# ethnhe/FFB6D

Hardware: AMD Instinct MI355X
Metric: RGB-D frames/sec fwd (480x640, N=12288, bs=8) (higher is better)
Workload: dtype f32; 1 GPU; FFB6D forward incl. on-device 22-call KNN index pyramid; bs=8/GPU, N=12288 pts, 480x640 RGB-D, 22 classes, fp32, eval; global_batch=8, n_points=12288, index_dtype=int64, layout=pm, parallelism=dp1 (independent batches, one process per GPU, no process group)

## Files before the change

### ffb6d_amd/_lib.py

```python
import ctypes
import os

from . import build as _build

_c = ctypes
_vp, _i64, _i32, _sz = _c.c_void_p, _c.c_int64, _c.c_int, _c.c_size_t

SIGNATURES = {
    "ffb6d_last_error": (_c.c_char_p, []),
    "ffb6d_abi_version": (_c.c_int, []),
    "cpp_knn": (None, [_vp, _sz, _sz, _vp, _sz, _sz, _vp]),
    "cpp_knn_omp": (None, [_vp, _sz, _sz, _vp, _sz, _sz, _vp]),
    "cpp_knn_batch": (None, [_vp, _sz, _sz, _sz, _vp, _sz, _sz, _vp]),
    "cpp_knn_batch_omp": (None, [_vp, _sz, _sz, _sz, _vp, _sz, _sz, _vp]),
    "cpp_knn_batch_distance_pick": (None, [_vp, _sz, _sz, _sz, _vp, _sz, _sz, _vp]),
    "cpp_knn_batch_distance_pick_omp": (None, [_vp, _sz, _sz, _sz, _vp, _sz, _sz, _vp]),
    "ffb6d_knn_workspace_bytes": (_sz, [_i64, _i64, _i64, _i32]),
    "ffb6d_knn_batch_device": (_i32, [_vp, _vp, _i64, _i64, _i64, _i32, _vp, _vp, _vp, _vp, _sz, _vp]),
    "ffb6d_knn_prepared_bytes": (_sz, [_i64, _i64]),
    "ffb6d_knn_prepare_workspace_bytes": (_sz, [_i64, _i64]),
    "ffb6d_knn_prepare": (_i32, [_vp, _i64, _i64, _vp, _sz, _vp, _sz, _vp]),
    "ffb6d_knn_prepare_multi_workspace_bytes": (_sz, [_i32, _vp, _i64]),
    "ffb6d_knn_prepare_multi": (_i32, [_i32, _vp, _vp, _i64, _vp, _vp, _vp, _sz, _vp]),
    "ffb6d_knn_search_multi": (_i32, [_i32, _vp, _i64, _vp]),
    "ffb6d_knn_search_prepared": (_i32, [_vp, _vp, _vp, _i64, _i64, _i64, _i32, _vp, _vp, _vp, _vp]),
    "ffb6d_knn_set_pair_counter": (_i32, [_vp]),
    "ffb6d_knn_uses_pruning": (_i32, [_i64, _i64, _i64, _i32]),
    "ffb6d_random_sample_f32": (_i32, [_vp, _vp, _i32, _vp, _vp, _i64, _i64, _i64, _i64, _i32, _vp]),
    "ffb6d_random_sample_bwd_f32": (_i32, [_vp, _vp, _vp, _i64, _i64, _i64, _i64, _vp]),
    "ffb6d_nearest_interpolation_f32": (_i32, [_vp, _vp, _i32, _vp, _i64, _i64, _i64, _i64, _vp]),
    "ffb6d_nearest_interpolation_bwd_f32": (_i32, [_vp, _vp, _i32, _vp, _i64, _i64, _i64, _i64, _vp]),
    "ffb6d_gather_neighbour_f32": (_i32, [_vp, _vp, _i32, _vp, _i64, _i64, _i64, _i64, _i32, _vp]),
    "ffb6d_gather_neighbour_bwd_f32": (_i32, [_vp, _vp, _i32, _vp, _i64, _i64, _i64, _i64, _i32, _vp]),
    "ffb6d_relative_pos_encoding_f32": (_i32, [_vp, _vp, _i32, _vp, _i64, _i64, _i32, _vp]),
    "ffb6d_att_pool_f32": (_i32, [_vp, _vp, _vp, _i64, _i64, _i64, _i32, _vp]),
    "ffb6d_relative_pos_encoding_cm_f32": (_i32, [_vp, _vp, _i32, _vp, _i64, _i64, _i32, _vp]),
    "ffb6d_att_pool_bwd_f32": (_i32, [_vp, _vp, _vp, _vp, _vp, _i64, _i64, _i64, _i32, _vp]),
    "ffb6d_mlp_pm_f32": (_i32, [_vp, _vp, _vp, _i64, _i64, _vp, _i64, _vp, _i64, _i64, _vp, _i64, _vp, _i64, _i32, _i64, _vp,
                                _i64, _i64, _i64, _i32, _i32, _vp]),
    "ffb6d_mlp_pm_tile": (_i32, [_i64, _i64, _i64, _i32]),
    "ffb6d_mlp_pm_choice": (_i32, [_i64, _i64, _i64, _i64, _i32, _i32, _i32]),
    "ffb6d_mlp_pm_seq_plan": (_i32, [_i64, _i64]),
    "ffb6d_mlp_pm_batched_f32": (_i32, [_vp, _i64, _i64, _vp, _i64, _i64, _vp, _i64, _i64, _i64, _i32, _vp]),
    "ffb6d_wino_input_f32": (_i32, [_vp, _vp, _i64, _i64, _i64, _i64, _i64, _vp]),
    "ffb6d_wino_output_f32": (_i32, [_vp, _vp, _vp, _vp, _vp, _vp, _vp, _i64, _i64, _i64, _i64, _i64, _i32, _c.c_float, _vp]),
    "ffb6d_wino4_input_f32": (_i32, [_vp, _vp, _i64, _i64, _i64, _i64, _i64, _vp]),
    "ffb6d_wino4_output_f32": (_i32, [_vp, _vp, _vp, _vp, _vp, _vp, _vp, _i64, _i64, _i64, _i64, _i64, _i32, _c.c_float, _vp]),
    "ffb6d_wino4_conv_f32": (_i32, [_vp, _vp, _vp, _vp, _vp, _vp, _vp, _vp, _i64, _i64, _i64, _i64, _i64, _i32, _c.c_float, _i32, _vp]),
    "ffb6d_wino4_conv_form": (_i32, [_i64, _i64]),
    "ffb6d_mlp_pm_set_big_form": (None, [_i32]),
    "ffb6d_mlp_pm_set_seq_lin": (None, [_i32]),
    "ffb6d_att_pool_pm_f32": (_i32, [_vp, _vp, _i64, _i64, _vp, _i32, _vp, _i64, _i64, _vp, _i64, _i64, _i64, _i32, _vp]),
    "ffb6d_mlp_pm_bf16": (_i32, [_vp, _vp, _vp, _i64, _i64, _vp, _i64, _vp, _i64, _i64, _vp, _i64, _vp, _i64, _i32, _i64, _vp,
                                 _i64, _i64, _i64, _i32, _i32, _vp]),
    "ffb6d_att_pool_pm_bf16": (_i32, [_vp, _vp, _i64, _i64, _vp, _i32, _vp, _i64, _i64, _vp, _i64, _i64, _i64, _i32, _vp]),
    "ffb6d_random_sample_pm": (_i32, [_i32, _vp, _vp, _i32, _vp, _i64, _i64, _i64, _i64, _i32, _vp]),
    "ffb6d_gather_rows_pm": (_i32, [_i32, _vp, _vp, _i32, _vp, _i64, _i64, _i64, _i64, _vp]),
    "ffb6d_relative_pos_encoding_pm": (_i32, [_i32, _vp, _vp, _i32, _vp, _i64, _i64, _i32, _vp]),
    "ffb6d_affine_act_pm": (_i32, [_i32, _vp, _vp, _vp, _vp, _vp, _vp, _vp, _i64, _i64, _i32, _c.c_float, _vp]),
    "ffb6d_affine_relu_maxpool_pm": (_i32, [_i32, _vp, _vp, _vp, _vp, _i64, _i64, _i64, _i64, _vp]),
    "ffb6d_bilinear_resize_pm": (_i32, [_i32, _vp, _vp, _i64, _i64, _i64, _i64, _i64, _i64, _i32, _vp]),
    "ffb6d_mlp_chain3_pm_f32": (_i32, [_vp, _i64, _vp, _vp, _i32, _vp, _vp, _i32, _vp, _vp, _i32, _vp, _i64, _i64, _i64, _vp]),
    "ffb6d_mlp_chain3_pm_bf16": (_i32, [_vp, _i64, _vp, _vp, _i32, _vp, _vp, _i32, _vp, _vp, _i32, _vp, _i64, _i64, _i64, _vp]),
    "ffb6d_upsampled_patch_rows_pm": (_i32, [_i32, _vp, _vp, _i32, _vp, _i64, _i64, _i64, _i64, _i64, _i64, _i64, _vp]),
    "ffb6d_posenc_mlp_pm": (_i32, [_i32, _vp, _vp, _i32, _vp, _i64, _vp, _i32, _vp, _i64, _i64, _i32, _i64, _vp]),
    "ffb6d_lfa_pm": (_i32, [_i32, _i32, _vp, _i64, _vp, _i32, _vp, _i64, _vp, _i64, _vp, _i32, _vp, _vp, _i32, _vp, _vp, _vp, _i32, _vp, _i64,
# ... 163 lines not shown
```

### ffb6d_amd/forward_pm.py

```python
import torch
import torch.nn.functional as F

from . import _lib, ops, ops_pm, pyramid


def cached(mod, name, sources, build):
    key = tuple((t._version, t.data_ptr(), t.device) for t in sources)
    store = mod.__dict__.setdefault("_pm_cache", {})
    hit = store.get(name)
    if hit is None or hit[0] != key:
        with torch.no_grad():
            hit = (key, build())
        store[name] = hit
    return hit[1]


def _pad_k(w, k_to):
    if w.shape[1] == k_to:
        return w.contiguous()
    out = w.new_zeros(w.shape[0], k_to)
    out[:, :w.shape[1]] = w
    return out


# ... 55 lines not shown


def mlp(m, x1, x2=None, pad_k=None, **kw):
    w, b = folded(m, pad_k, x1.dtype)
    return ops_pm.mlp(x1, w, b, m.act_code, x2=x2, **kw)


def fc_weight(att, dt=F32):
    w = att.fc.weight
    return cached(att, "fc%s" % dt, [w], lambda: w.detach().reshape(w.shape[0], -1).to(dt).contiguous())


POSENC_FUSED = True
STEM_FUSED = True
LFA_FUSED = True
HEADS_SHARE_FIRST = True
HEADS_ALIGN_LAST = True
HEADS_ON_BOTH_STREAMS = True
HEADS_CHAIN_FUSED = True
GEMM_SEQ_FORM = True
GEMM_BIG_FORM = True
GEMM_SEQ_LIN = False
GEMM_SEQ_LIN_ONE = False
LFA_WIDTHS = (32, 64, 128, 256)


def folded_kc(m, dt, perm=False):
    def build():
        w, b = folded(m, dt=dt)
        return ops_pm.k_chunked(w, perm), b
    return cached(m, "kc%s%d" % (dt, perm), mlp_sources(m), build)


def building_block(bb, xyz, f_pc, nei):
    dt = f_pc.dtype
    if LFA_FUSED and 2 * f_pc.shape[-1] in LFA_WIDTHS and nei.shape[-1] == 16:
        w1, b1 = folded(bb.mlp1)
        a1, a2 = bb.att_pooling_1, bb.att_pooling_2
        wm1, bm1 = folded_kc(a1.mlp, dt)
        f_agg = ops_pm.lfa_half(1, xyz, nei, f_pc, w1, b1, bb.mlp1.act_code, fc_weight(a1, dt), wm1, bm1, a1.mlp.act_code)
        w2, b2 = folded(bb.mlp2, dt=dt)
        wm2, bm2 = folded_kc(a2.mlp, dt)
        return ops_pm.lfa_half(2, xyz, nei, f_agg, w1, b1, bb.mlp1.act_code, fc_weight(a2, dt), wm2, bm2, a2.mlp.act_code,
                               w2=w2, b2=b2, act2=bb.mlp2.act_code)
    if xyz.shape[-1] == 4:
        xyz = xyz[..., :3].contiguous()
# ... 20 lines not shown
    w, b = cached(rb, "res%d%s" % (kin, dt), mlp_sources(rb.mlp2) + mlp_sources(rb.shortcut), build)
    return ops_pm.mlp(f, w, b, ops.ACT_LEAKY, x2=feature)


def decode(stage, skip, p_emb, interp_idx):
    wa, wb, bias = split(stage, skip.shape[-1], skip.dtype)
    y = ops_pm.mlp(p_emb, wb)
    return ops_pm.mlp(skip, wa, bias, stage.act_code, gather=(y, interp_idx.reshape(interp_idx.shape[0], -1)))


def fusion_step(pre_p2r, fuse_p2r, pre_r2p, fuse_r2p, rgb0, p0, p2r_idx, r2p_idx, main=None, side=None, handover=None, tag=""):
    B, h, w_, c = rgb0.shape
    if main is None:
        main = side = torch.cuda.current_stream(rgb0.device)
    if handover is None:
        handover = lambda t, producer, consumer, tag=None: t
    handover(p0, side, main, "main waits for point stage " + tag)
    handover(rgb0, main, side, "side waits for colour stage " + tag)
    if side is not main:
        p2r_idx.record_stream(main)
    e = mlp(pre_p2r, p0)
    wa, wb, bias = split(fuse_p2r, c, rgb0.dtype)
    y = ops_pm.mlp(e, wb)
    rgb = ops_pm.mlp(rgb0, wa, bias, fuse_p2r.act_code, gather=(y, p2r_idx.reshape(B, -1)))
    with torch.cuda.stream(side):
        r2p = mlp(pre_r2p, ops_pm.random_sample(rgb0.view(B, h * w_, c), r2p_idx))
        p = mlp(fuse_r2p, p0, x2=r2p)
    return rgb, p


def conv(x, c):
    w = cached(c, "cl%s" % x.dtype, [c.weight],
               lambda: c.weight.detach().to(x.dtype).contiguous(memory_format=torch.channels_last))
    y = F.conv2d(x.permute(0, 3, 1, 2), w, None, c.stride, c.padding, c.dilation, c.groups)
    y = y.permute(0, 2, 3, 1)
    return y if y.is_contiguous() else y.contiguous()


TRUNK_WINOGRAD = True
TRUNK_WINOGRAD_MIN_CIN = 256


def wino_filter(w):
    G = torch.tensor([[1, 0, 0], [.5, .5, .5], [.5, -.5, .5], [0, 0, 1]], dtype=torch.float64, device=w.device)
    u = G @ w.detach().double() @ G.T
    return u.permute(2, 3, 0, 1).reshape(16, w.shape[0], w.shape[1]).float().contiguous()


def wino_weights(c):
    return cached(c, "wino", [c.weight], lambda: wino_filter(c.weight))


TRUNK_WINOGRAD_F4 = True


def wino4_filter(w):
    G = torch.tensor([[1 / 2, 0, 0], [-1 / 6, -1 / 6, -1 / 6], [1 / 6, -1 / 6, 1 / 6], [1 / 30, 1 / 15, 2 / 15],
                      [-16 / 15, 8 / 15, -4 / 15], [0, 0, 1 / 2]], dtype=torch.float64, device=w.device)
    u = G @ w.detach().double() @ G.T
    return u.permute(2, 3, 0, 1).reshape(36, w.shape[0], w.shape[1]).float().contiguous()


def wino4_weights(c):
    return cached(c, "wino4", [c.weight], lambda: wino4_filter(c.weight))


def wino_variant(B, H, W):
    if not TRUNK_WINOGRAD_F4:
        return 2
    return 4 if 36 * ops_pm.wino4_tiles(B, H, W)[1] < 16 * ops_pm.wino_tiles(B, H, W)[1] else 2


def wino_ok(c, x, m=None):
    if not TRUNK_WINOGRAD or x.dtype != torch.float32 or c.weight.dtype != torch.float32:
        return False
    if (c.kernel_size, c.stride, c.padding, c.dilation, c.groups) != ((3, 3), (1, 1), (1, 1), (1, 1), 1) or c.bias is not None \
            or c.padding_mode != "zeros":
        return False
    cout, cin = c.weight.shape[:2]
    if cin < TRUNK_WINOGRAD_MIN_CIN or cin < 128 or cin % 32 or cout % 4:
        return False
    B, H, W, _ = x.shape
    if m is None:
        m = wino_variant(B, H, W)
    planes, Tp = (m + 2) ** 2, (ops_pm.wino4_tiles if m == 4 else ops_pm.wino_tiles)(B, H, W)[1]
    lim = (1 << 31) - (1 << 20)
    return planes * (Tp + 256) * max(cin, cout) * 4 < lim and B * H * W * max(cin, cout) * 4 < lim and planes * cout * cin * 4 < lim


def conv_wino(x, c, scale, shift, residual=None, res_affine=None, m=None):
    if m is None:
        m = wino_variant(*x.shape[:3])
    x = x if x.is_contiguous() else x.contiguous()
    if m == 4:
        mm = ops_pm.mlp_batched(ops_pm.wino4_input(x), wino4_weights(c))
        return ops_pm.wino4_output(mm, x.shape[:3], scale, shift, act=ops.ACT_RELU, residual=residual, res_affine=res_affine)
    if m != 2:
        raise ValueError(f"conv_wino: m must be 2, 4 or None, got {m}")
    u = wino_weights(c)
    v = ops_pm.wino_input(x)
    mm = ops_pm.mlp_batched(v, u)
    return ops_pm.wino_output(mm, x.shape[:3], scale, shift, act=ops.ACT_RELU, residual=residual, res_affine=res_affine)


TRUNK_WINOGRAD_FUSED = True
TRUNK_WINOGRAD_FUSED_WIDTHS = frozenset({(64, 64), (128, 128), (128, 256)})


def wino_fused_ok(c, x):
    if not (TRUNK_WINOGRAD and TRUNK_WINOGRAD_FUSED) or x.dtype != torch.float32 or c.weight.dtype != torch.float32:
        return False
    if (c.kernel_size, c.stride, c.padding, c.dilation, c.groups) != ((3, 3), (1, 1), (1, 1), (1, 1), 1) or c.bias is not None \
            or c.padding_mode != "zeros":
        return False
    cout, cin = c.weight.shape[:2]
    if (cin, cout) not in TRUNK_WINOGRAD_FUSED_WIDTHS or cin not in ops_pm.WINO4_CONV_CIN or cout not in ops_pm.WINO4_CONV_COUT:
        return False
    B, H, W, _ = x.shape
# ... 31 lines not shown
        return conv_wino(y, rb.conv2, *ops.bn_fold(rb.bn2), residual=res, res_affine=res_affine)
    return ops_pm.affine_act_(y, *ops.bn_fold(rb.bn2), act=ops.ACT_RELU, residual=res, res_affine=res_affine)


def pyramid_pooling(pp, x):
    B, h, w_, C = x.shape
    sizes = [st[0].output_size[0] for st in pp.stages]
    bw = pp.bottleneck.weight

    def build():
        ch = pp.stages[0][1].weight.shape[0]
        wb = bw.detach().reshape(bw.shape[0], -1)
        prods = [(wb[:, i * ch:(i + 1) * ch] @ st[1].weight.detach().reshape(ch, ch)).contiguous()
                 for i, st in enumerate(pp.stages)]
        return prods, wb[:, len(pp.stages) * ch:].contiguous()
    prods, wx = cached(pp, "fold", [bw] + [st[1].weight for st in pp.stages], build)
    pooled = ops_pm.psp_pool(x, sizes)
    zs, off = [], 0
    for s, wl in zip(sizes, prods):
        zs.append(ops_pm.mlp(pooled[:, off:off + s * s].contiguous(), wl, role="cnn"))
        off += s * s
    prior = ops_pm.psp_prior_sum(torch.cat(zs, dim=1), sizes, (h, w_), dtype=x.dtype)
    wx = cached(pp, "wx%s" % x.dtype, [bw], lambda: wx.to(x.dtype))
    return ops_pm.mlp(x, wx, pp.bottleneck.bias.detach().float(), ops.ACT_RELU, add=prior, role="cnn")


UPCONV_FOLD = "auto"
UPCONV_FOLD_BF16 = True


def _fold_block(cin, dtype):
    if UPCONV_FOLD == "auto":
        return dtype == torch.float32 or UPCONV_FOLD_BF16
    return UPCONV_FOLD is None or cin in UPCONV_FOLD


def upconv_folded(ub, dt=F32):
    cv, bn, prelu = ub.conv[1], ub.conv[2], ub.conv[3]
    if prelu.weight.numel() != 1:
        raise NotImplementedError("per-channel PReLU in PSPUpsample")

    def build():
        scale = bn.weight.detach() * torch.rsqrt(bn.running_var + bn.eps)
        shift = bn.bias.detach() - bn.running_mean * scale
        if cv.bias is not None:
            shift = shift + scale * cv.bias.detach()
        w = cv.weight.detach() * scale[:, None, None, None]
        w9 = w.permute(2, 3, 0, 1).reshape(9 * w.shape[0], w.shape[1])
        return w9.to(dt).contiguous(), shift.float().contiguous(), float(prelu.weight.detach().item())
    src = [cv.weight, bn.weight, bn.bias, bn.running_mean, bn.running_var, prelu.weight] + ([cv.bias] if cv.bias is not None else [])
    return cached(ub, "fold9%s" % dt, src, build)


def up_block(ub, x):
    B, h, w_, cin = x.shape
    cv, bn, prelu = ub.conv[1], ub.conv[2], ub.conv[3]
    if _fold_block(cin, x.dtype) and cv.kernel_size == (3, 3) and cv.padding == (1, 1) \
            and cv.stride == (1, 1) and cv.dilation == (1, 1) and cv.groups == 1:
        w9, shift, slope = upconv_folded(ub, x.dtype)
        z = ops_pm.mlp(x, w9, role="cnn")
        return ops_pm.upconv_combine(z, shift, slope, (2 * h, 2 * w_))
    y = ops_pm.bilinear_resize(x, (2 * h, 2 * w_), align_corners=True)
    y = conv(y, cv)
    if prelu.weight.numel() != 1:
        raise NotImplementedError("per-channel PReLU in PSPUpsample")
    slope = cached(ub, "slope", [prelu.weight], lambda: float(prelu.weight.detach().item()))
    scale, shift = ops.bn_fold(bn)
    shift = cached(ub, "shift", [cv.bias, bn.weight, bn.bias, bn.running_mean, bn.running_var],
                   lambda: (shift + scale * cv.bias.detach()).contiguous())
    return ops_pm.affine_act_(y, scale, shift, act=ops.ACT_LEAKY, slope=slope)


def final_head(fh, x):
    cv = fh[0]
    w = cached(fh, "w%s" % x.dtype, [cv.weight], lambda: cv.weight.detach().reshape(cv.out_channels, -1).to(x.dtype).contiguous())
    return ops_pm.mlp(x, w, cv.bias.detach().float(), ops_pm.ACT_LOG_SOFTMAX, role="cnn")


LAST_STAGE_AT_CHOSEN = True


def last_stage_at_chosen(stage, x, choose):
    from . import model
# ... 284 lines not shown
```

### ffb6d_amd/ops_pm.py

```python
import torch

from . import _lib
from .ops import ACT_LEAKY, ACT_NONE, ACT_RELU, _idx, _need_gpu, _stream


def _dt(*ts):
    dts = {t.dtype for t in ts if t is not None}
    if len(dts) != 1 or next(iter(dts)) not in (torch.float32, torch.bfloat16):
        raise TypeError(f"row operands must all be float32 or all bfloat16, got {sorted(map(str, dts))}")
    return 1 if next(iter(dts)) == torch.bfloat16 else 0


def rows_view(x):
    C = x.shape[-1]
    x2 = x.reshape(-1, C)
    if x2.stride(1) != 1 or x2.data_ptr() % 16 or (x2.shape[0] > 1 and (x2.stride(0) * x2.element_size()) % 16):
        x2 = x2.contiguous()
    return x2, (x2.stride(0) if x2.shape[0] > 1 else C)


ACT_LOG_SOFTMAX = 3
MLP_SEQ_FORM = True
MLP_BIG_FORM = True
MLP_SEQ_LIN = 0
_big_form_set = _seq_lin_set = None


def _sync_big_form(lib):
    global _big_form_set, _seq_lin_set
    if _big_form_set is not MLP_BIG_FORM:
        lib.ffb6d_mlp_pm_set_big_form(int(MLP_BIG_FORM))
        _big_form_set = MLP_BIG_FORM
    if _seq_lin_set != MLP_SEQ_LIN:
        lib.ffb6d_mlp_pm_set_seq_lin(int(MLP_SEQ_LIN))
        _seq_lin_set = MLP_SEQ_LIN


def mlp(x1, w, bias=None, act=ACT_NONE, x2=None, add=None, gather=None, x1_gather=None, out=None, tile_hint=0, role="path"):
    _need_gpu(x1, w)
    lib = _lib.load()
    _sync_big_form(lib)
    dt = _dt(x1, w, x2, add, gather[0] if gather is not None else None, out)
    tdt = x1.dtype
    esz = x1.element_size()
    if bias is not None and bias.dtype != torch.float32:
        raise TypeError("bias stays float32 in both precisions")
    a, ld1 = rows_view(x1.detach())
    K1 = a.shape[1]
    xi, px, bits = None, 0, 0
    lead = x1.shape[:-1]
    if x1_gather is not None:
        if x1.dim() != 3 or x1_gather.dim() != 2 or x1_gather.shape[0] != x1.shape[0]:
            raise ValueError("x1_gather needs x1 [B,M,K1] and idx [B,P]")
        xi, bits = _idx(x1_gather.reshape(-1))
        px = x1.shape[1]
        lead = tuple(x1_gather.shape)
    rows = 1
    for n in lead:
        rows *= int(n)
    P = rows // lead[0] if (x1_gather is not None or gather is not None) and len(lead) else rows
    b, ld2, K2 = None, 0, 0
# ... 19 lines not shown
        if gi.numel() != rows or rows % B:
            raise ValueError("gather index must have one entry per output row")
        P = rows // B
    elif add is not None:
        y, ldy = rows_view(add.detach())
        if y.shape[0] != rows or y.shape[1] != Cout:
            raise ValueError(f"add {tuple(add.shape)} does not match the output [{rows}, {Cout}]")
    if out is None:
        out = torch.empty(tuple(lead) + (Cout,), dtype=tdt, device=x1.device)
    if out.stride(-1) != 1 or out.numel() != rows * Cout:
        raise ValueError("out must be [..., Cout] with contiguous channels")
    ldo = out.stride(-2) if out.dim() >= 2 and rows > 1 else Cout
    if out.dim() > 2 and any(out.stride(i) != out.stride(i + 1) * out.shape[i + 1] for i in range(out.dim() - 2)):
        raise ValueError("out must be row-regular (a channel slice of a contiguous row buffer is fine)")
    nbytes = esz * ((K1 + K2) * Cout + rows * (K1 + K2) + rows * Cout) + rows * (bits // 8) * ((gi is not None) + (xi is not None)) + \
        (esz * (y.shape[0] if gi is None else rows) * Cout if y is not None else 0)
    if tile_hint == 0 and not MLP_SEQ_FORM and not dt and \
            (lib.ffb6d_mlp_pm_choice(rows, Cout, K1, K2, int(act), 0, int(xi is not None)) & 255) == 8:
        tile_hint = 7
    if _lib.TRACER is not None:
        tile = (int(tile_hint) if tile_hint > 0 else lib.ffb6d_mlp_pm_choice(rows, Cout, K1, K2, int(act), int(dt), int(xi is not None))) & 255
    else:
        tile = 0
    with torch.cuda.device(x1.device), _lib.traced("mlp_pm", nbytes, (K1 + K2, Cout, rows, tile, dt, role)):
        rc = (lib.ffb6d_mlp_pm_bf16 if dt else lib.ffb6d_mlp_pm_f32)(w.data_ptr(), bias.data_ptr() if bias is not None else None,
                                  a.data_ptr(), K1, ld1, xi.data_ptr() if xi is not None else None, px,
                                  b.data_ptr() if b is not None else None, K2, ld2,
                                  y.data_ptr() if y is not None else None, ldy,
                                  gi.data_ptr() if gi is not None else None, py, bits, P,
                                  out.data_ptr(), ldo, rows, Cout, int(act), int(tile_hint), _stream(x1))
    _lib.check(rc, "ffb6d_mlp_pm_f32")
    return out


def mlp_batched(x, w, out=None, tile_hint=0):
    _need_gpu(x, w)
    lib = _lib.load()
    if x.dtype != torch.float32 or w.dtype != torch.float32 or (out is not None and out.dtype != torch.float32):
        raise TypeError("mlp_batched is float32 only")
    if x.dim() != 3 or w.dim() != 3 or w.shape[0] != x.shape[0] or w.shape[2] != x.shape[2] or not x.is_contiguous() or not w.is_contiguous():
        raise ValueError(f"mlp_batched needs contiguous x [G,R,K] and w [G,Cout,K], got {tuple(x.shape)} / {tuple(w.shape)}")
    G, R, K = x.shape
    Cout = w.shape[1]
    if out is None:
        out = torch.empty(G, R, Cout, dtype=torch.float32, device=x.device)
    if out.shape != (G, R, Cout) or not out.is_contiguous():
        raise ValueError("out must be contiguous [G, R, Cout]")
    if tile_hint == 0 and not MLP_SEQ_FORM:
        tile_hint = 7
    nbytes = 4 * G * (Cout * K + R * K + R * Cout)
    with torch.cuda.device(x.device), _lib.traced("mlp_pm_batched", nbytes, (K, Cout, G * R, (int(tile_hint) & 255) or 8, 0, "cnn")):
        rc = lib.ffb6d_mlp_pm_batched_f32(w.data_ptr(), Cout * K, R, x.data_ptr(), K, K, out.data_ptr(), Cout, G * R, Cout,
                                          int(tile_hint), _stream(x))
    _lib.check(rc, "ffb6d_mlp_pm_batched_f32")
    return out


def wino_tiles(B, H, W):
    T = B * ((H + 1) // 2) * ((W + 1) // 2)
    return T, -(-T // 128) * 128


def wino_input(x, out=None):
    _need_gpu(x)
    lib = _lib.load()
    if x.dtype != torch.float32 or x.dim() != 4 or not x.is_contiguous():
        raise ValueError("wino_input needs a contiguous float32 [B,H,W,C] map")
    B, H, W, C = x.shape
    T, Tp = wino_tiles(B, H, W)
    if out is None:
        out = torch.empty(16, Tp, C, dtype=torch.float32, device=x.device)
    if out.shape != (16, Tp, C) or not out.is_contiguous() or out.dtype != torch.float32:
        raise ValueError(f"out must be contiguous float32 [16, {Tp}, {C}]")
# ... 417 lines not shown
```

### include/ffb6d_ops.h

```cpp
#ifndef FFB6D_OPS_H_
#define FFB6D_OPS_H_

#include "ffb6d_knn.h"

#ifdef __cplusplus
extern "C" {
#endif

int ffb6d_random_sample_f32(const float* feat, const void* idx, int idx_bits,
                            float* out, int32_t* arg,
                            int64_t B, int64_t C, int64_t M, int64_t Np, int K,
                            ffb6d_stream_t stream);

int ffb6d_random_sample_bwd_f32(const float* grad_out, const int32_t* arg, float* grad_feat,
                                int64_t B, int64_t C, int64_t M, int64_t Np,
                                ffb6d_stream_t stream);

int ffb6d_nearest_interpolation_f32(const float* feat, const void* idx, int idx_bits,
                                    float* out,
                                    int64_t B, int64_t C, int64_t M, int64_t U,
                                    ffb6d_stream_t stream);

int ffb6d_nearest_interpolation_bwd_f32(const float* grad_out, const void* idx, int idx_bits,
                                        float* grad_feat,
// ... 30 lines not shown

int ffb6d_depth_normal(const void* depth_mm, int depth_is_u16, double fx, double fy, int kernel_size,
                       int distance_threshold, int difference_threshold, int point_into_surface, float* out, int64_t B,
                       int64_t H, int64_t W, ffb6d_stream_t stream);

size_t ffb6d_fill_missing_workspace_bytes(int64_t B, int64_t H, int64_t W);
int ffb6d_fill_missing_f32(const float* depth, double cam_scale, double scale_2_80m, float max_depth, float* out, int64_t B,
                           int64_t H, int64_t W, void* workspace, size_t workspace_bytes, ffb6d_stream_t stream);


int ffb6d_mlp_pm_f32(const float* w, const float* bias, const float* x1, int64_t k1, int64_t ld1, const void* x1_idx,
                     int64_t x1_rows_per_frame, const float* x2, int64_t k2, int64_t ld2, const float* y, int64_t ldy,
                     const void* y_idx, int64_t y_rows_per_frame, int idx_bits, int64_t rows_per_frame, float* out,
                     int64_t ldo, int64_t rows, int64_t cout, int act, int tile_hint, ffb6d_stream_t stream);

int ffb6d_mlp_pm_tile(int64_t rows, int64_t cout, int64_t K, int act);
int ffb6d_mlp_pm_choice(int64_t rows, int64_t cout, int64_t k1, int64_t k2, int act, int bf16, int x1_gathered);
int ffb6d_mlp_pm_seq_plan(int64_t rows, int64_t cout);
void ffb6d_mlp_pm_set_seq_lin(int on);
void ffb6d_mlp_pm_set_big_form(int on);

int ffb6d_mlp_pm_batched_f32(const float* w, int64_t w_stride, int64_t rows_per_w, const float* x, int64_t k, int64_t ld, float* out,
                             int64_t ldo, int64_t rows, int64_t cout, int tile_hint, ffb6d_stream_t stream);

int ffb6d_wino_input_f32(const float* x, float* v, int64_t B, int64_t H, int64_t W, int64_t C, int64_t Tp, ffb6d_stream_t stream);
int ffb6d_wino_output_f32(const float* m, const float* scale, const float* shift, const float* res, const float* rscale,
                          const float* rshift, float* out, int64_t B, int64_t H, int64_t W, int64_t O, int64_t Tp, int act, float slope,
                          ffb6d_stream_t stream);

int ffb6d_wino4_input_f32(const float* x, float* v, int64_t B, int64_t H, int64_t W, int64_t C, int64_t Tp, ffb6d_stream_t stream);
int ffb6d_wino4_output_f32(const float* m, const float* scale, const float* shift, const float* res, const float* rscale,
                           const float* rshift, float* out, int64_t B, int64_t H, int64_t W, int64_t O, int64_t Tp, int act, float slope,
                           ffb6d_stream_t stream);

int ffb6d_wino4_conv_f32(const float* x, const float* u, const float* scale, const float* shift, const float* res, const float* rscale,
                         const float* rshift, float* out, int64_t B, int64_t H, int64_t W, int64_t C, int64_t O, int act, float slope,
                         int form, ffb6d_stream_t stream);
int ffb6d_wino4_conv_form(int64_t C, int64_t O);

int ffb6d_att_pool_pm_f32(const float* w_fc, const float* f, int64_t c1, int64_t ldf, const void* nei, int idx_bits,
                          const float* g, int64_t c2, int64_t ldg, float* out, int64_t ldo, int64_t B, int64_t N, int K,
                          ffb6d_stream_t stream);

int ffb6d_mlp_pm_bf16(const void* w, const float* bias, const void* x1, int64_t k1, int64_t ld1, const void* x1_idx,
                      int64_t x1_rows_per_frame, const void* x2, int64_t k2, int64_t ld2, const void* y, int64_t ldy,
                      const void* y_idx, int64_t y_rows_per_frame, int idx_bits, int64_t rows_per_frame, void* out,
// ... 74 lines not shown
```

Measured before the change: 646.8 frames/s.

## Add split-bf16 (bf16x3) MFMA GEMM form for large fp32 pointwise and Winograd layers

Adds a new GEMM kernel that emulates fp32 matrix multiplies with three bf16 splits of each operand and six bf16 MFMA products, so fp32 layers can use the bf16 matrix cores. Weight splits are precomputed and cached per module. The activation split happens on the fly while staging into LDS, with double-buffered LDS DMA for the weights. It is routed to large-row layers (p2r fusion, PSP bottleneck, folded upconv, Winograd-4 batched GEMM) only where the existing chooser would pick tile 8. Dropping the lowest-order cross terms costs a little accuracy relative to true fp32, and the kernel uses a large LDS footprint.

```diff
diff --git a/ffb6d_amd/_lib.py b/ffb6d_amd/_lib.py
--- a/ffb6d_amd/_lib.py
+++ b/ffb6d_amd/_lib.py
@@ -42,6 +42,10 @@
     "ffb6d_mlp_pm_choice": (_i32, [_i64, _i64, _i64, _i64, _i32, _i32, _i32]),
     "ffb6d_mlp_pm_seq_plan": (_i32, [_i64, _i64]),
     "ffb6d_mlp_pm_batched_f32": (_i32, [_vp, _i64, _i64, _vp, _i64, _i64, _vp, _i64, _i64, _i64, _i32, _vp]),
+    "ffb6d_mlp_pm_split_w": (_i32, [_vp, _vp, _i64, _vp]),
+    "ffb6d_mlp_pm_split_f32": (_i32, [_vp, _vp, _vp, _i64, _i64, _vp, _i64, _vp, _i64, _i64, _vp, _i64, _vp, _i64, _i32, _i64, _vp,
+                                      _i64, _i64, _i64, _i32, _i32, _vp]),
+    "ffb6d_mlp_pm_split_batched_f32": (_i32, [_vp, _i64, _i64, _vp, _i64, _i64, _vp, _i64, _i64, _i64, _vp]),
     "ffb6d_wino_input_f32": (_i32, [_vp, _vp, _i64, _i64, _i64, _i64, _i64, _vp]),
     "ffb6d_wino_output_f32": (_i32, [_vp, _vp, _vp, _vp, _vp, _vp, _vp, _i64, _i64, _i64, _i64, _i64, _i32, _c.c_float, _vp]),
     "ffb6d_wino4_input_f32": (_i32, [_vp, _vp, _i64, _i64, _i64, _i64, _i64, _vp]),
diff --git a/ffb6d_amd/csrc/mlp_pm_split.hip b/ffb6d_amd/csrc/mlp_pm_split.hip
--- /dev/null
+++ b/ffb6d_amd/csrc/mlp_pm_split.hip
@@ -0,0 +1,297 @@
+#include <algorithm>
+
+#include "common.h"
+#include "ffb6d_ops.h"
+#include "mlp_pm_common.h"
+
+namespace ffb6d {
+namespace pm {
+namespace {
+
+constexpr int SP_BLK = 512;
+constexpr int SP_RB = 64;
+constexpr int SP_WIMG = 256 * SP_RB;
+constexpr int SP_XIMG = 128 * SP_RB;
+constexpr int SP_XBASE = 3 * SP_WIMG;
+constexpr int SP_STAGE = 3 * SP_WIMG + 3 * SP_XIMG;
+constexpr int SP_LDS = 2 * SP_STAGE;
+static_assert(SP_LDS <= 160 * 1024, "LDS layout");
+
+typedef __bf16 bf16x2 __attribute__((ext_vector_type(2)));
+
+__device__ __forceinline__ void split3(float a, __bf16& a0, __bf16& a1, __bf16& a2)
+{
+    a0 = (__bf16)a;
+    const float r1 = a - (float)a0;
+    a1 = (__bf16)r1;
+    a2 = (__bf16)(r1 - (float)a1);
+}
+
+__global__ void __launch_bounds__(256) split_w_kernel(const float* __restrict__ w, __bf16* __restrict__ w3, long long n)
+{
+    for (long long e = blockIdx.x * 256LL + threadIdx.x; e < n; e += 256LL * gridDim.x) {
+        __bf16 a0, a1, a2;
+        split3(w[e], a0, a1, a2);
+        w3[e] = a0;
+        w3[n + e] = a1;
+        w3[2 * n + e] = a2;
+    }
+}
+
+template <int VAR>
+__global__ void __launch_bounds__(SP_BLK)
+mlp_pm_split_kernel(const PmParams p, const unsigned part_bytes)
+{
+    constexpr int OOB = 0x7ffffff0;
+    extern __shared__ __attribute__((aligned(16))) unsigned char lds[];
+
+    const int t = blockIdx.x;
+    const int xcd = t & 7, sl = t >> 3;
+    const int pt = (sl / p.n_ct) * 8 + xcd;
+    const int ct = sl % p.n_ct;
+    if (pt >= p.n_pt) return;
+    const int r0 = pt * 128, c0 = ct * 256;
+
+    const int lane = threadIdx.x & 63;
+    const int l31 = lane & 31, kh = lane >> 5;
+    const int wave = __builtin_amdgcn_readfirstlane(threadIdx.x >> 6);
+    const int wm = wave >> 2, wn = wave & 3;
+    const int K = p.k1;
+    const int nstep = K / 32;
+    const int wrow0 = p.rows_per_w ? (r0 / p.rows_per_w) * p.cout : 0;
+
+    const unsigned char* w3 = static_cast<const unsigned char*>(p.w);
+    const __amdgpu_buffer_rsrc_t rs_w[3] = {make_rsrc(w3, part_bytes), make_rsrc(w3 + part_bytes, part_bytes),
+                                            make_rsrc(w3 + 2 * (size_t)part_bytes, part_bytes)};
+    const __amdgpu_buffer_rsrc_t rs_x = make_rsrc(p.x1, span_bytes((unsigned)p.rows, p.ld1, p.k1, 4));
+
+    const int lrow = 16 * wave + (lane >> 2);
+    const int lchunk = ((lane & 3) ^ ((lrow >> 3) & 3)) * 16;
+    int w_off[2];
+#pragma unroll
+    for (int h = 0; h < 2; ++h) {
+        const int ch = c0 + 128 * h + lrow;
+        w_off[h] = ch < p.cout ? (wrow0 + ch) * (K * 2) + lchunk : OOB;
+    }
+    auto request_w = [&](int s, int stage) {
+        unsigned char* wi = lds + stage * SP_STAGE + wave * (16 * SP_RB);
+#pragma unroll
+        for (int pi = 0; pi < 3; ++pi)
+#pragma unroll
+            for (int h = 0; h < 2; ++h) lds_dma16(rs_w[pi], wi + pi * SP_WIMG + h * (128 * SP_RB), w_off[h], s * SP_RB);
+    };
+
+    const int xrow = threadIdx.x >> 2, xq = threadIdx.x & 3;
+    const bool xlive = r0 + xrow < p.rows;
+    const int x_off0 = xlive ? (r0 + xrow) * p.ld1 * 4 + xq * 32 : OOB;
+    const int x_off1 = xlive ? x_off0 + 16 : OOB;
+    const int x_dst = SP_XBASE + xrow * SP_RB + ((xq ^ ((xrow >> 3) & 3)) * 16);
+    auto load_x = [&](int s, u32x4 (&v)[2]) {
+        v[0] = __builtin_amdgcn_raw_buffer_load_b128(rs_x, x_off0, s * 128, 0);
+        v[1] = __builtin_amdgcn_raw_buffer_load_b128(rs_x, x_off1, s * 128, 0);
+    };
+    auto write_x = [&](int stage, const u32x4 (&v)[2]) {
+        u32x4 o[3];
+        if constexpr (VAR & 1) {
+#pragma unroll
+            for (int q = 0; q < 4; ++q) {
+                const unsigned pk = (v[q >> 1][2 * (q & 1)] >> 16) | (v[q >> 1][2 * (q & 1) + 1] & 0xffff0000u);
+                o[0][q] = pk; o[1][q] = 0u; o[2][q] = 0u;
+            }
+        } else {
+#pragma unroll
+            for (int q = 0; q < 4; ++q) {
+                bf16x2 b0, b1, b2;
+                __bf16 s0, s1, s2;
+                split3(__uint_as_float(v[q >> 1][2 * (q & 1)]), s0, s1, s2);
+                b0[0] = s0; b1[0] = s1; b2[0] = s2;
+                split3(__uint_as_float(v[q >> 1][2 * (q & 1) + 1]), s0, s1, s2);
+                b0[1] = s0; b1[1] = s1; b2[1] = s2;
+                o[0][q] = __builtin_bit_cast(unsigned, b0);
+                o[1][q] = __builtin_bit_cast(unsigned, b1);
+                o[2][q] = __builtin_bit_cast(unsigned, b2);
+            }
+        }
+        unsigned char* xi = lds + stage * SP_STAGE + x_dst;
+#pragma unroll
+        for (int pj = 0; pj < 3; ++pj) *reinterpret_cast<u32x4*>(xi + pj * SP_XIMG) = o[pj];
+    };
+
+    const int fsw = (l31 >> 3) & 3;
+    const int a_row = (wm * 128 + l31) * SP_RB, b_row = SP_XBASE + (wn * 32 + l31) * SP_RB;
+    f32x16 acc[4][1];
+#pragma unroll
+    for (int i = 0; i < 4; ++i)
+#pragma unroll
+        for (int r = 0; r < 16; ++r) acc[i][0][r] = 0.f;
+
+    auto multiply = [&](int stage, int ks) {
+        const unsigned char* im = lds + stage * SP_STAGE;
+        const int fo = ((2 * ks + kh) ^ fsw) * 16;
+        u32x4 a[3][4], b[3];
+#pragma unroll
+        for (int pj = 0; pj < 3; ++pj) b[pj] = *reinterpret_cast<const u32x4*>(im + b_row + pj * SP_XIMG + fo);
+#pragma unroll
+        for (int pi = 0; pi < 3; ++pi)
+#pragma unroll
+            for (int i = 0; i < 4; ++i) a[pi][i] = *reinterpret_cast<const u32x4*>(im + pi * SP_WIMG + a_row + i * (32 * SP_RB) + fo);
+        if constexpr (VAR & 2) {
+#pragma unroll
+            for (int pi = 0; pi < 3; ++pi)
+#pragma unroll
+                for (int i = 0; i < 4; ++i) use_here(a[pi][i][0] ^ b[pi][3]);
+            return;
+        }
+        constexpr int TW[6] = {0, 1, 2, 0, 1, 0}, TX[6] = {2, 1, 0, 1, 0, 0};
+#pragma unroll
+        for (int tm = 0; tm < 6; ++tm)
+#pragma unroll
+            for (int i = 0; i < 4; ++i)
+                acc[i][0] = __builtin_amdgcn_mfma_f32_32x32x16_bf16(__builtin_bit_cast(bf16x8, a[TW[tm]][i]),
+                                                                   __builtin_bit_cast(bf16x8, b[TX[tm]]), acc[i][0], 0, 0, 0);
+    };
+
+    {
+        u32x4 xv[2];
+        request_w(0, 0);
+        load_x(0, xv);
+        write_x(0, xv);
+    }
+    __syncthreads();
+    for (int s = 0; s < nstep; ++s) {
+        const int st = s & 1;
+        const bool more = s + 1 < nstep;
+        u32x4 xv[2];
+        if (more) {
+            request_w(s + 1, st ^ 1);
+            load_x(s + 1, xv);
+        }
+        __builtin_amdgcn_sched_barrier(0);
+        multiply(st, 0);
+        __builtin_amdgcn_sched_barrier(0);
+        if (more) write_x(st ^ 1, xv);
+        __builtin_amdgcn_sched_barrier(0);
+        multiply(st, 1);
+        __builtin_amdgcn_sched_barrier(0);
+        lds_dma_wait<0>();
+        __syncthreads();
+    }
+    if constexpr (VAR & 4) {
+        if (p.act != 77) return;
+    }
+    pm_epilogue<float, 4, 1, false>(p, acc, c0, r0, wm, wn, l31, kh);
+}
+
+template <int VAR>
+bool launch_split(PmParams& p, unsigned part_bytes, hipStream_t st)
+{
+    static int attr_set[kMaxDevices + 1];
+    const int slot = device_slot();
+    if (!cache_get(attr_set, slot)) {
+        if (hipFuncSetAttribute(reinterpret_cast<const void*>(&mlp_pm_split_kernel<VAR>), hipFuncAttributeMaxDynamicSharedMemorySize, SP_LDS) !=
+            hipSuccess)
+            return false;
+        cache_set(attr_set, slot, 1);
+    }
+    p.n_ct = (int)ceil_div(p.cout, 256);
+    p.n_pt = (int)ceil_div(p.rows, 128);
+    const unsigned grid = (unsigned)(ceil_div(p.n_pt, 8) * 8 * p.n_ct);
+    hipLaunchKernelGGL(mlp_pm_split_kernel<VAR>, dim3(grid), dim3(SP_BLK), SP_LDS, st, p, part_bytes);
+    return true;
+}
+
+bool split_form_ok(const PmParams& p, int64_t w_rows, int64_t y_rows)
+{
+    const int64_t K = p.k1;
+    return p.k2 == 0 && !p.x2 && !p.xidx && p.act >= 0 && p.act <= 2 && K % 32 == 0 && K >= 64 && (p.cout & 3) == 0 &&
+           (p.ld1 & 3) == 0 && ((reinterpret_cast<uintptr_t>(p.x1) | reinterpret_cast<uintptr_t>(p.w)) & 15) == 0 &&
+           ((int64_t)p.rows + 256) * p.ld1 * 4 < (1LL << 31) && ((int64_t)p.rows + 256) * p.ldo * 4 < (1LL << 31) &&
+           (w_rows + 256) * K * 2 < (1LL << 31) && (!p.y || (y_rows + 256) * p.ldy * 4 < (1LL << 31));
+}
+
+}
+}
+}
+
+using namespace ffb6d;
+using namespace ffb6d::pm;
+
+extern "C" int ffb6d_mlp_pm_split_w(const float* w, void* w3, int64_t n, ffb6d_stream_t stream)
+{
+    FFB6D_REQUIRE(n >= 0, "mlp_pm_split_w: bad size");
+    if (n == 0) return FFB6D_OK;
+    FFB6D_REQUIRE(w && w3, "mlp_pm_split_w: null pointer");
+    const unsigned grid = (unsigned)std::min<int64_t>(ceil_div(n, 256), 4096);
+    hipLaunchKernelGGL(split_w_kernel, dim3(grid), dim3(256), 0, as_stream(stream), w, static_cast<__bf16*>(w3), (long long)n);
+    FFB6D_LAUNCH_CHECK();
+    return FFB6D_OK;
+}
+
+extern "C" int ffb6d_mlp_pm_split_f32(const void* w3, const float* bias, const float* x1, int64_t k1, int64_t ld1, const void* x1_idx,
+                                      int64_t x1_rows_per_frame, const float* x2, int64_t k2, int64_t ld2, const float* y, int64_t ldy,
+                                      const void* y_idx, int64_t y_rows_per_frame, int idx_bits, int64_t rows_per_frame, float* out,
+                                      int64_t ldo, int64_t rows, int64_t cout, int act, int variant, ffb6d_stream_t stream)
+{
+    (void)x1_rows_per_frame; (void)ld2;
+    FFB6D_REQUIRE(rows >= 0 && cout >= 1 && k1 >= 1 && k2 >= 0, "mlp_pm_split: bad shape");
+#ifndef FFB6D_SPLIT_PROBES
+    FFB6D_REQUIRE(variant == 0, "mlp_pm_split: the library carries variant 0 only");
+#endif
+    if (rows == 0) return FFB6D_OK;
+    FFB6D_REQUIRE(w3 && x1 && out, "mlp_pm_split: null pointer");
+    FFB6D_REQUIRE(ld1 >= k1 && ldo >= cout, "mlp_pm_split: row stride smaller than the row");
+    FFB6D_REQUIRE(!y_idx || y, "mlp_pm_split: gather indices without rows to gather");
+    FFB6D_REQUIRE(!y_idx || ((idx_bits == 32 || idx_bits == 64) && rows_per_frame >= 1 && rows % rows_per_frame == 0 && y_rows_per_frame >= 1),
+                  "mlp_pm_split: index arrays need idx_bits 32/64 and rows_per_frame dividing rows");
+    FFB6D_REQUIRE(!y || ldy >= cout, "mlp_pm_split: ldy smaller than cout");
+    PmParams p;
+    p.w = w3; p.bias = bias; p.x1 = x1; p.xidx = x1_idx; p.x2 = x2; p.y = y; p.gidx = y_idx; p.out = out;
+    p.rows = (int)rows; p.cout = (int)cout; p.k1 = (int)k1; p.k2 = (int)k2; p.ld1 = (int)ld1; p.ld2 = 4;
+    p.ldy = (int)ldy; p.ldo = (int)ldo; p.P = (int)(y_idx ? rows_per_frame : rows); p.py = (int)y_rows_per_frame; p.px = 0;
+    p.act = act; p.idx64 = idx_bits == 64;
+    const int64_t y_rows = y ? (y_idx ? rows / rows_per_frame * y_rows_per_frame : rows) : 0;
+    FFB6D_REQUIRE(rows < (1LL << 31) && cout < (1LL << 31) && k1 < (1LL << 31) && ld1 < (1LL << 31) && ldo < (1LL << 31) && ldy < (1LL << 31) &&
+                  split_form_ok(p, cout, y_rows),
+                  "mlp_pm_split: the split-bf16 form needs one ungathered fp32 source with K %% 32 == 0, K >= 64, cout %% 4 == 0, "
+                  "16-byte aligned operand rows, act 0..2 and buffers under 2 GiB");
+    const unsigned part_bytes = (unsigned)(cout * k1 * 2);
+    bool ok;
+    switch (variant) {
+#ifdef FFB6D_SPLIT_PROBES
+        case 1: ok = launch_split<1>(p, part_bytes, as_stream(stream)); break;
+        case 2: ok = launch_split<2>(p, part_bytes, as_stream(stream)); break;
+        case 4: ok = launch_split<4>(p, part_bytes, as_stream(stream)); break;
+        case 6: ok = launch_split<6>(p, part_bytes, as_stream(stream)); break;
+#endif
+        default: ok = launch_split<0>(p, part_bytes, as_stream(stream)); break;
+    }
+    if (!ok)
+        return set_error(FFB6D_ERR_HIP, "mlp_pm_split: hipFuncSetAttribute(MaxDynamicSharedMemorySize) failed");
+    FFB6D_LAUNCH_CHECK();
+    return FFB6D_OK;
+}
+
+extern "C" int ffb6d_mlp_pm_split_batched_f32(const void* w3, int64_t n_w, int64_t rows_per_w, const float* x, int64_t k, int64_t ld,
+                                              float* out, int64_t ldo, int64_t rows, int64_t cout, ffb6d_stream_t stream)
+{
+    FFB6D_REQUIRE(rows >= 0 && cout >= 1 && k >= 1 && n_w >= 1, "mlp_pm_split_batched: bad shape");
+    FFB6D_REQUIRE(rows_per_w >= 128 && rows_per_w % 128 == 0 && rows_per_w < (1LL << 31),
+                  "mlp_pm_split_batched: rows_per_w must be a positive multiple of 128 (got %lld): a point tile multiplies one matrix",
+                  (long long)rows_per_w);
+    if (rows == 0) return FFB6D_OK;
+    FFB6D_REQUIRE(w3 && x && out, "mlp_pm_split_batched: null pointer");
+    FFB6D_REQUIRE(ld >= k && ldo >= cout && ceil_div(rows, rows_per_w) <= n_w, "mlp_pm_split_batched: stride smaller than the row, or more "
+                  "rows than matrices");
+    PmParams p;
+    p.w = w3; p.bias = nullptr; p.x1 = x; p.xidx = nullptr; p.x2 = nullptr; p.y = nullptr; p.gidx = nullptr; p.out = out;
+    p.rows = (int)rows; p.cout = (int)cout; p.k1 = (int)k; p.k2 = 0; p.ld1 = (int)ld; p.ld2 = 4; p.ldy = 0; p.ldo = (int)ldo;
+    p.P = (int)rows; p.py = 0; p.px = 0; p.act = 0; p.idx64 = 0;
+    p.rows_per_w = (int)rows_per_w; p.w_stride = (int)(cout * k);
+    FFB6D_REQUIRE(rows < (1LL << 31) && cout < (1LL << 31) && k < (1LL << 31) && ld < (1LL << 31) && ldo < (1LL << 31) &&
+                  n_w * cout < (1LL << 31) && split_form_ok(p, n_w * cout, 0),
+                  "mlp_pm_split_batched: needs K %% 32 == 0, K >= 64, cout %% 4 == 0, 16-byte aligned rows and buffers under 2 GiB");
+    if (!launch_split<0>(p, (unsigned)(n_w * cout * k * 2), as_stream(stream)))
+        return set_error(FFB6D_ERR_HIP, "mlp_pm_split_batched: hipFuncSetAttribute(MaxDynamicSharedMemorySize) failed");
+    FFB6D_LAUNCH_CHECK();
+    return FFB6D_OK;
+}
diff --git a/ffb6d_amd/forward_pm.py b/ffb6d_amd/forward_pm.py
--- a/ffb6d_amd/forward_pm.py
+++ b/ffb6d_amd/forward_pm.py
@@ -101,6 +101,19 @@
 GEMM_BIG_FORM = True
 GEMM_SEQ_LIN = False
 GEMM_SEQ_LIN_ONE = False
+GEMM_SPLIT_FORM = True
+
+
+def gemm_split_takes(rows, cout, K, act=0):
+    return GEMM_SPLIT_FORM and K % 32 == 0 and K >= 256 and cout >= 256 and cout % 4 == 0 and rows >= 32768 and 0 <= int(act) <= 2 and \
+        (_lib.load().ffb6d_mlp_pm_choice(rows, cout, K, 0, int(act), 0, 0) & 255) == 8
+
+
+def mlp_long(owner, key, sources, x, w, bias=None, act=ops.ACT_NONE, **kw):
+    if x.dtype == F32 and gemm_split_takes(x.numel() // x.shape[-1], w.shape[0], w.shape[1], act):
+        w3 = cached(owner, "w3" + key, sources, lambda: ops_pm.split_weight(w))
+        return ops_pm.mlp(x, w, bias, act, tile_hint=ops_pm.SPLIT_FORM, w_split=w3, **kw)
+    return ops_pm.mlp(x, w, bias, act, **kw)
 LFA_WIDTHS = (32, 64, 128, 256)
 
 
@@ -167,7 +180,7 @@
     e = mlp(pre_p2r, p0)
     wa, wb, bias = split(fuse_p2r, c, rgb0.dtype)
     y = ops_pm.mlp(e, wb)
-    rgb = ops_pm.mlp(rgb0, wa, bias, fuse_p2r.act_code, gather=(y, p2r_idx.reshape(B, -1)))
+    rgb = mlp_long(fuse_p2r, "p2r%d" % c, mlp_sources(fuse_p2r), rgb0, wa, bias, fuse_p2r.act_code, gather=(y, p2r_idx.reshape(B, -1)))
     with torch.cuda.stream(side):
         r2p = mlp(pre_r2p, ops_pm.random_sample(rgb0.view(B, h * w_, c), r2p_idx))
         p = mlp(fuse_r2p, p0, x2=r2p)
@@ -208,6 +221,10 @@
 
 def wino4_weights(c):
     return cached(c, "wino4", [c.weight], lambda: wino4_filter(c.weight))
+
+
+def wino4_split_weights(c):
+    return cached(c, "wino4_3", [c.weight], lambda: ops_pm.split_weight(wino4_weights(c)))
 
 
 def wino_variant(B, H, W):
@@ -238,7 +255,11 @@
         m = wino_variant(*x.shape[:3])
     x = x if x.is_contiguous() else x.contiguous()
     if m == 4:
-        mm = ops_pm.mlp_batched(ops_pm.wino4_input(x), wino4_weights(c))
+        v, u = ops_pm.wino4_input(x), wino4_weights(c)
+        if gemm_split_takes(v.shape[0] * v.shape[1], u.shape[1], u.shape[2]):
+            mm = ops_pm.mlp_batched(v, u, tile_hint=ops_pm.SPLIT_FORM, w_split=wino4_split_weights(c))
+        else:
+            mm = ops_pm.mlp_batched(v, u)
         return ops_pm.wino4_output(mm, x.shape[:3], scale, shift, act=ops.ACT_RELU, residual=residual, res_affine=res_affine)
     if m != 2:
         raise ValueError(f"conv_wino: m must be 2, 4 or None, got {m}")
@@ -316,7 +337,7 @@
         off += s * s
     prior = ops_pm.psp_prior_sum(torch.cat(zs, dim=1), sizes, (h, w_), dtype=x.dtype)
     wx = cached(pp, "wx%s" % x.dtype, [bw], lambda: wx.to(x.dtype))
-    return ops_pm.mlp(x, wx, pp.bottleneck.bias.detach().float(), ops.ACT_RELU, add=prior, role="cnn")
+    return mlp_long(pp, "wx", [bw], x, wx, pp.bottleneck.bias.detach().float(), ops.ACT_RELU, add=prior, role="cnn")
 
 
 UPCONV_FOLD = "auto"
@@ -342,8 +363,12 @@
         w = cv.weight.detach() * scale[:, None, None, None]
         w9 = w.permute(2, 3, 0, 1).reshape(9 * w.shape[0], w.shape[1])
         return w9.to(dt).contiguous(), shift.float().contiguous(), float(prelu.weight.detach().item())
-    src = [cv.weight, bn.weight, bn.bias, bn.running_mean, bn.running_var, prelu.weight] + ([cv.bias] if cv.bias is not None else [])
-    return cached(ub, "fold9%s" % dt, src, build)
+    return cached(ub, "fold9%s" % dt, upconv_sources(ub), build)
+
+
+def upconv_sources(ub):
+    cv, bn, prelu = ub.conv[1], ub.conv[2], ub.conv[3]
+    return [cv.weight, bn.weight, bn.bias, bn.running_mean, bn.running_var, prelu.weight] + ([cv.bias] if cv.bias is not None else [])
 
 
 def up_block(ub, x):
@@ -352,7 +377,7 @@
     if _fold_block(cin, x.dtype) and cv.kernel_size == (3, 3) and cv.padding == (1, 1) \
             and cv.stride == (1, 1) and cv.dilation == (1, 1) and cv.groups == 1:
         w9, shift, slope = upconv_folded(ub, x.dtype)
-        z = ops_pm.mlp(x, w9, role="cnn")
+        z = mlp_long(ub, "fold9", upconv_sources(ub), x, w9, role="cnn")
         return ops_pm.upconv_combine(z, shift, slope, (2 * h, 2 * w_))
     y = ops_pm.bilinear_resize(x, (2 * h, 2 * w_), align_corners=True)
     y = conv(y, cv)
diff --git a/ffb6d_amd/ops_pm.py b/ffb6d_amd/ops_pm.py
--- a/ffb6d_amd/ops_pm.py
+++ b/ffb6d_amd/ops_pm.py
@@ -36,7 +36,31 @@
         _seq_lin_set = MLP_SEQ_LIN
 
 
-def mlp(x1, w, bias=None, act=ACT_NONE, x2=None, add=None, gather=None, x1_gather=None, out=None, tile_hint=0, role="path"):
+def split_weight(w):
+    _need_gpu(w)
+    if w.dtype != torch.float32:
+        raise TypeError("split_weight takes a float32 weight")
+    w = w.detach().contiguous()
+    w3 = torch.empty((3,) + tuple(w.shape), dtype=torch.bfloat16, device=w.device)
+    with torch.cuda.device(w.device):
+        rc = _lib.load().ffb6d_mlp_pm_split_w(w.data_ptr(), w3.data_ptr(), w.numel(), _stream(w))
+    _lib.check(rc, "ffb6d_mlp_pm_split_w")
+    return w3
+
+
+SPLIT_FORM = 10
+
+
+def _split_images(w, w_split):
+    if w_split is None:
+        w_split = split_weight(w)
+    if w_split.dtype != torch.bfloat16 or tuple(w_split.shape) != (3,) + tuple(w.shape) or not w_split.is_contiguous():
+        raise ValueError(f"w_split must be contiguous bfloat16 [3, {', '.join(map(str, w.shape))}] (split_weight(w))")
+    return w_split
+
+
+def mlp(x1, w, bias=None, act=ACT_NONE, x2=None, add=None, gather=None, x1_gather=None, out=None, tile_hint=0, role="path",
+        w_split=None):
     _need_gpu(x1, w)
     lib = _lib.load()
     _sync_big_form(lib)
@@ -102,6 +126,19 @@
         tile = (int(tile_hint) if tile_hint > 0 else lib.ffb6d_mlp_pm_choice(rows, Cout, K1, K2, int(act), int(dt), int(xi is not None))) & 255
     else:
         tile = 0
+    if tile_hint == SPLIT_FORM:
+        if dt:
+            raise TypeError("the split-bf16 form (tile_hint 10) takes float32 rows")
+        w3 = _split_images(w, w_split)
+        with torch.cuda.device(x1.device), _lib.traced("mlp_pm", nbytes, (K1 + K2, Cout, rows, tile, dt, role)):
+            rc = lib.ffb6d_mlp_pm_split_f32(w3.data_ptr(), bias.data_ptr() if bias is not None else None,
+                                            a.data_ptr(), K1, ld1, xi.data_ptr() if xi is not None else None, px,
+                                            b.data_ptr() if b is not None else None, K2, ld2,
+                                            y.data_ptr() if y is not None else None, ldy,
+                                            gi.data_ptr() if gi is not None else None, py, bits, P,
+                                            out.data_ptr(), ldo, rows, Cout, int(act), 0, _stream(x1))
+        _lib.check(rc, "ffb6d_mlp_pm_split_f32")
+        return out
     with torch.cuda.device(x1.device), _lib.traced("mlp_pm", nbytes, (K1 + K2, Cout, rows, tile, dt, role)):
         rc = (lib.ffb6d_mlp_pm_bf16 if dt else lib.ffb6d_mlp_pm_f32)(w.data_ptr(), bias.data_ptr() if bias is not None else None,
                                   a.data_ptr(), K1, ld1, xi.data_ptr() if xi is not None else None, px,
@@ -113,7 +150,7 @@
     return out
 
 
-def mlp_batched(x, w, out=None, tile_hint=0):
+def mlp_batched(x, w, out=None, tile_hint=0, w_split=None, rows=None):
     _need_gpu(x, w)
     lib = _lib.load()
     if x.dtype != torch.float32 or w.dtype != torch.float32 or (out is not None and out.dtype != torch.float32):
@@ -129,6 +166,17 @@
     if tile_hint == 0 and not MLP_SEQ_FORM:
         tile_hint = 7
     nbytes = 4 * G * (Cout * K + R * K + R * Cout)
+    if tile_hint == SPLIT_FORM:
+        w3 = _split_images(w, w_split)
+        n_rows = G * R if rows is None else int(rows)
+        if not 0 <= n_rows <= G * R:
+            raise ValueError(f"rows must lie in [0, {G * R}]")
+        with torch.cuda.device(x.device), _lib.traced("mlp_pm_batched", nbytes, (K, Cout, n_rows, SPLIT_FORM, 0, "cnn")):
+            rc = lib.ffb6d_mlp_pm_split_batched_f32(w3.data_ptr(), G, R, x.data_ptr(), K, K, out.data_ptr(), Cout, n_rows, Cout, _stream(x))
+        _lib.check(rc, "ffb6d_mlp_pm_split_batched_f32")
+        return out
+    if rows is not None:
+        raise ValueError("rows is an argument of the split-bf16 form (tile_hint 10)")
     with torch.cuda.device(x.device), _lib.traced("mlp_pm_batched", nbytes, (K, Cout, G * R, (int(tile_hint) & 255) or 8, 0, "cnn")):
         rc = lib.ffb6d_mlp_pm_batched_f32(w.data_ptr(), Cout * K, R, x.data_ptr(), K, K, out.data_ptr(), Cout, G * R, Cout,
                                           int(tile_hint), _stream(x))
diff --git a/include/ffb6d_ops.h b/include/ffb6d_ops.h
--- a/include/ffb6d_ops.h
+++ b/include/ffb6d_ops.h
@@ -76,6 +76,14 @@
 
 int ffb6d_mlp_pm_batched_f32(const float* w, int64_t w_stride, int64_t rows_per_w, const float* x, int64_t k, int64_t ld, float* out,
                              int64_t ldo, int64_t rows, int64_t cout, int tile_hint, ffb6d_stream_t stream);
+
+int ffb6d_mlp_pm_split_w(const float* w, void* w3, int64_t n, ffb6d_stream_t stream);
+int ffb6d_mlp_pm_split_f32(const void* w3, const float* bias, const float* x1, int64_t k1, int64_t ld1, const void* x1_idx,
+                           int64_t x1_rows_per_frame, const float* x2, int64_t k2, int64_t ld2, const float* y, int64_t ldy,
+                           const void* y_idx, int64_t y_rows_per_frame, int idx_bits, int64_t rows_per_frame, float* out, int64_t ldo,
+                           int64_t rows, int64_t cout, int act, int variant, ffb6d_stream_t stream);
+int ffb6d_mlp_pm_split_batched_f32(const void* w3, int64_t n_w, int64_t rows_per_w, const float* x, int64_t k, int64_t ld, float* out,
+                                   int64_t ldo, int64_t rows, int64_t cout, ffb6d_stream_t stream);
 
 int ffb6d_wino_input_f32(const float* x, float* v, int64_t B, int64_t H, int64_t W, int64_t C, int64_t Tp, ffb6d_stream_t stream);
 int ffb6d_wino_output_f32(const float* m, const float* scale, const float* shift, const float* res, const float* rscale,
```

Result: faster. 726.0 frames/s (median of 6 runs) (+12.2%).
